# sriram-0311/MC-SLAM

Measured on AMD Instinct MI355X. Metric: multi-cam frames/sec (4-cam 1280x720 @2000 kpts/cam, extract + intra-rig match), higher is better.
Workload: dtype u8; 1 GPU; 4-cam rig 1280x720, 2000 kpts/cam, extract + all-pairs intra-rig match (configs[1]); slots=4, frames_per_launch=128, cameras=4, nfeatures=2000

## Files before the change

mc-slam_amd/csrc/mcorb_device.h:

```cpp
#pragma once
#include <hip/hip_runtime.h>
#include <stdint.h>

#include "mcorb_common.h"

namespace mcorb {

typedef short s16x2 __attribute__((ext_vector_type(2)));
typedef unsigned short u16x2 __attribute__((ext_vector_type(2)));
typedef int v4i __attribute__((ext_vector_type(4)));

__device__ __forceinline__ int lane_id() { return threadIdx.x & 63; }
__device__ __forceinline__ int lane_rank(unsigned long long mask, int acc = 0)
{
    return (int)__builtin_amdgcn_mbcnt_hi((uint32_t)(mask >> 32), __builtin_amdgcn_mbcnt_lo((uint32_t)mask, (uint32_t)acc));
}
__device__ __forceinline__ int wave_uniform(int v) { return __builtin_amdgcn_readfirstlane(v); }
__device__ __forceinline__ void wave_lds_sync()
{
    __builtin_amdgcn_fence(__ATOMIC_RELEASE, "workgroup");
    __builtin_amdgcn_wave_barrier();
    __builtin_amdgcn_fence(__ATOMIC_ACQUIRE, "workgroup");
}
__device__ __forceinline__ int xcd_remap(int b, int n)
{
    const int q = n >> 3, r = n & 7, x = b & 7;
    return (x < r ? x * (q + 1) : r * (q + 1) + (x - r) * q) + (b >> 3);
}
__device__ __forceinline__ int reflect101(int p, int len)
{
    if (p < 0) p = -p;
    if (p >= len) p = 2 * len - 2 - p;
    return p;
}

struct UndistScales {
    float s[kMaxLevels];
    UndistScales(const float *scale, int nlevels) : s{}
    {
        for (int l = 0; l < nlevels && l < kMaxLevels; l++) s[l] = scale[l];
    }
};
__device__ __forceinline__ float2 sel_point(uint32_t v, const UndistScales &sc)
{
    int l, xl, yl;
    unpack_sel(v, l, xl, yl);
    float x = (float)xl, y = (float)yl;
    if (l != 0) { x *= sc.s[l]; y *= sc.s[l]; }
    return make_float2(x, y);
}

__device__ __forceinline__ uint32_t bcnt_acc(uint32_t x, uint32_t acc)
{
    uint32_t r;
    asm("v_bcnt_u32_b32 %0, %1, %2" : "=v"(r) : "v"(x), "v"(acc));
    return r;
}
__device__ __forceinline__ uint32_t hamming256(const ulonglong4 &a, const ulonglong4 &b)
{
    const unsigned long long x0 = a.x ^ b.x, x1 = a.y ^ b.y, x2 = a.z ^ b.z, x3 = a.w ^ b.w;
    uint32_t d = __builtin_popcount((uint32_t)x0);
    d = bcnt_acc((uint32_t)(x0 >> 32), d);
    d = bcnt_acc((uint32_t)x1, d);
    d = bcnt_acc((uint32_t)(x1 >> 32), d);
    d = bcnt_acc((uint32_t)x2, d);
    d = bcnt_acc((uint32_t)(x2 >> 32), d);
    d = bcnt_acc((uint32_t)x3, d);
    d = bcnt_acc((uint32_t)(x3 >> 32), d);
    return d;
}

}
```

mc-slam_amd/csrc/mcorb_engine.cpp:

```cpp
#include <stdlib.h>
#include <string.h>
#include <sys/prctl.h>
#include <time.h>

#include "mcorb_engine.h"
#include "mcorb_prof.h"

namespace mcorb {

static thread_local std::string g_err;
void set_error(const std::string &msg) { g_err = msg; }
const char *get_error() { return g_err.c_str(); }
hipError_t Rig::wait_event(hipEvent_t ev) const
{
    if (wait_mode != 2) return hipEventSynchronize(ev);
    for (int i = 0;; i++) {
        const hipError_t e = hipEventQuery(ev);
        if (e != hipErrorNotReady) return e;
        if (i < 4) { std::this_thread::yield(); continue; }
        timespec ts = {0, 20000};
        nanosleep(&ts, nullptr);
    }
}

// ... 452 lines not shown
        std::vector<mcorb_keypoint> &K = s.kps[m];
        K.assign(total, mcorb_keypoint{});
        uint32_t *sel = s.hc.sel + (size_t)m * geom.kcap;
        int monoIndex = 0, stereoIndex = total - 1;
        if (total) {
            for (int l = 0; l < L; l++) {
                for (const uint32_t c : s.sel_val[(size_t)m * L + l]) {
                    const int xl = cand_x(c) + kMinBorder, yl = cand_y(c) + kMinBorder;
                    const mcorb_keypoint kp = make_keypoint(l, xl, yl, (float)cand_resp(c), 0.f);
                    int pos;
                    if (kp.x >= (float)j.lap0 && kp.x <= (float)j.lap1) pos = stereoIndex--;
                    else pos = monoIndex++;
                    K[pos] = kp;
                    sel[pos] = pack_sel(l, xl, yl);
                }
            }
        }
        s.mono[m] = monoIndex;
        s.hc.nsel[m] = total;
    }, pool_threads + s.index);
    if (bad.load() == 3) { set_error("internal: quad-tree went below the bucketing without the candidate list"); (void)hipStreamSynchronize(s.st); return MCORB_E_STATE; }
    if (bad.load() == 1) { set_error("selection failed: level too tall"); (void)hipStreamSynchronize(s.st); return MCORB_E_SIZE; }
    if (bad.load()) { set_error("keypoint capacity exceeded"); (void)hipStreamSynchronize(s.st); return MCORB_E_CAP; }
    const auto t1 = std::chrono::steady_clock::now();
    s.timing[T_SELECT] = std::chrono::duration<float, std::micro>(t1 - t0).count();
    LatProf::mark(3);

    s.nimg_done = nimg;
    if (then_match) TRY(prepare_match(s, j));
    TRY(enqueue_back(s, j, then_match, false));
    HIPCHK(hipEventRecord(s.ev_done, s.st));
    LatProf::mark(4);
    HIPCHK(wait_event(s.ev_done));
    if (!s.host_results) HIPCHK(wait_event(s.ev_side));
    LatProf::mark(5);
    if (params.orientation)
        for (int m = 0; m < nimg; m++)
            for (size_t k = 0; k < s.kps[m].size(); k++) s.kps[m][k].angle = s.h_angles[(size_t)m * geom.kcap + k];
    read_timing(s, s.host_results ? nullptr : s.ev_c);
    return MCORB_OK;
}

int Rig::enqueue_back(Slot &s, const Job &j, bool then_match, bool gpu_sel)
{
    const int nimg = j.nimg;
    const bool small = s.host_results, ev_on = s.ev_on();
    if (!gpu_sel && !small) HIPCHK(hipMemcpyAsync(s.d_ctrl, s.h_ctrl, s.ctrl_bytes, hipMemcpyHostToDevice, s.st));
    if (ev_on) HIPCHK(hipEventRecord(s.ev_desc0, s.st));
    if (small && undist_on) {
        HIPCHK(hipEventRecord(s.ubuf.ev_u0, s.st));
        HIPCHK(hipStreamWaitEvent(s.st_dma, s.ubuf.ev_u0, 0));
        TRY(enqueue_undistort(s, nimg));
    }
    launch_describe(s.st, s.d_pyr, blur_planes ? s.d_blur : nullptr, geom, s.ctl.sel, s.ctl.nsel, params.orientation, s.d_desc, s.d_angles, nimg,
                    small ? s.h_desc : nullptr);
    if (ev_on) HIPCHK(hipEventRecord(s.ev_desc1, s.st));
    if (small) {
        if (then_match) TRY(enqueue_match(s, j, true));
        HIPCHK(hipGetLastError());
        if (undist_on) HIPCHK(hipStreamWaitEvent(s.st, s.ubuf.ev_u1, 0));
        if (s.bow_job) TRY(enqueue_bow(s, nimg));
        if (gpu_sel && ev_on) HIPCHK(hipEventRecord(s.ev_side, s.st));
        return MCORB_OK;
    }
    const size_t nk = (size_t)nimg * geom.kcap;
    HIPCHK(hipStreamWaitEvent(s.st_dma, s.ev_desc1, 0));
    if (!copy_kernel) HIPCHK(hipMemcpyAsync(s.h_desc, s.d_desc, nk * 32, hipMemcpyDeviceToHost, s.st_dma));
    else launch_copy_to_host(s.st_dma, s.d_desc, s.h_desc, nk * 32);
    if (gpu_sel) {
        HIPCHK(hipMemcpyAsync(s.h_ctrl + s.ctrl_nsel_off, s.d_ctrl + s.ctrl_nsel_off, s.ctrl_pairs_end - s.ctrl_nsel_off + nk * sizeof(uint32_t),
                              hipMemcpyDeviceToHost, s.st_dma));
        HIPCHK(hipMemcpyAsync(s.h_res, s.d_res, s.res_resp_off + nk, hipMemcpyDeviceToHost, s.st_dma));
    }
    if (params.orientation) HIPCHK(hipMemcpyAsync(s.h_angles, s.d_angles, nk * sizeof(float), hipMemcpyDeviceToHost, s.st_dma));
    if (undist_on) TRY(enqueue_undistort(s, nimg));
    if (s.bow_job) TRY(enqueue_bow(s, nimg));
    if (then_match) TRY(enqueue_match(s, j, true));
    HIPCHK(hipGetLastError());
    HIPCHK(hipEventRecord(s.ev_side, s.st_dma));
    return MCORB_OK;
}

int Rig::enqueue_gpu_job(Slot &s, const Job &j, bool then_match)
{
    const int nimg = j.nimg;
    (void)hipGetLastError();
    const bool small = s.host_results, ev_on = s.ev_on();
    if (then_match && !small)
        HIPCHK(hipMemcpyAsync(s.d_ctrl, s.h_ctrl, s.ctrl_pairs_end, hipMemcpyHostToDevice, s.st));
    int *d_flags = reinterpret_cast<int *>(s.d_res.get());
    if (!small) HIPCHK(hipMemsetAsync(d_flags, 0, 16 * sizeof(int), s.st));
    TRY(enqueue_front(s, nimg, s.d_tbl));
    HIPCHK(launch_select(s.st, s.d_tbl, s.d_sorted, geom, s.d_selval, s.d_selcnt, d_flags, nimg, select_deep_cap, select_prof));
    launch_assemble(s.st, s.d_selval, s.d_selcnt, geom, tab.scale, j.lap0, j.lap1, s.dc.sel, s.d_res + s.res_resp_off, s.dc.nsel,
                    reinterpret_cast<int *>(s.d_res + s.res_mono_off), d_flags, nimg, small ? s.hc.sel : nullptr,
                    small ? s.h_res + s.res_resp_off : nullptr, small ? s.h_sig : nullptr);
    if (ev_on) HIPCHK(hipEventRecord(s.ev_s, s.st));
    if (ev_on) HIPCHK(hipEventRecord(s.ev_tables, s.st));
    if (blur_planes) launch_blur(s.st, s.d_pyr, s.d_blur, geom, nimg);
    if (ev_on) HIPCHK(hipEventRecord(s.ev_blur, s.st));
    return enqueue_back(s, j, then_match, true);
}

void Rig::gpu_job_begin()
{
    if (!gpu_job_limit) return;
    std::unique_lock<std::mutex> lk(gpu_jobs_m);
    gpu_jobs_cv.wait(lk, [this] { return gpu_jobs_running < gpu_job_limit; });
    gpu_jobs_running++;
}
void Rig::gpu_job_end()
{
    if (!gpu_job_limit) return;
    {
        std::lock_guard<std::mutex> lk(gpu_jobs_m);
        gpu_jobs_running--;
    }
    gpu_jobs_cv.notify_one();
}

int Rig::run_gpu_selected(Slot &s, const Job &j, bool then_match)
{
    TRY(begin_extract(s, j));
    const int nimg = j.nimg;
    s.nimg_done = nimg;
    if (then_match) TRY(prepare_match(s, j));
    if (s.host_results)
        for (int m = 0; m < nimg; m++) static_cast<volatile unsigned long long *>(s.h_sig)[m] = 0;
    auto records = [&](int m) {
        const int n = s.hc.nsel[m];
// ... 124 lines not shown
```

mc-slam_amd/csrc/mcorb_engine.h:

```cpp
#pragma once
#include <hip/hip_runtime.h>
#include <stdint.h>

#include <algorithm>
#include <atomic>
#include <condition_variable>
#include <functional>
#include <memory>
#include <mutex>
#include <string>
#include <thread>
#include <vector>

#include "../../include/mcorb.h"
#include "mcorb_common.h"
#include "mcorb_hip.h"
#include "mcorb_kernels.h"
#include "mcorb_select.h"

namespace mcorb {

const char *get_error();

struct Tables {
// ... 284 lines not shown
    int set_undistortion(int cam, const double *K, const double *dist, int ncoeffs);
    int undist_records(Slot &s, int m0, int n, std::vector<const mcorb_keypoint *> &out);
    int undist_default(Slot &s, int m0, int n, std::vector<const mcorb_keypoint *> &out);
    int max_pairs() const { return std::max(1, npp * max_frames); }

    std::vector<UndistImageCam> imgud_cams;
    std::vector<uint8_t> imgud_set;
    std::vector<std::vector<int16_t>> imgud_map1;
    std::vector<std::vector<uint16_t>> imgud_map2;
    std::vector<DevBuf<int16_t>> d_imgud_map1;
    std::vector<DevBuf<uint16_t>> d_imgud_map2;
    DevBuf<RemapCam> d_remap_cams;
    bool imgud_on = false;
    int set_image_undistortion(int cam, const double *K, const double *dist, int ncoeffs);
    int enqueue_remap(Slot &s, int nimg);

    struct BowBinding {
        int flags = 0, levelsup = 0, L = 0, weighting = 0, scoring = 0;
        double ratio = 0.85;
        const int *child_start = nullptr, *child_count = nullptr, *child_id = nullptr, *word_id = nullptr;
        const void *child_desc = nullptr;
        const double *weight = nullptr;
    };
    BowBinding bow_bind;
    unsigned bow_gen = 0;
    bool lf_on = false;
    int lf_total_feats = 3000;
    std::vector<mcorb_camera> lf_cams;
    DevBuf<LfCam> d_lfcams;
    unsigned lf_gen = 0;
    int set_lf(const mcorb_camera *cams, int total_feats);
    int set_vocabulary(const BowBinding &b);
    int check_job_shape(const Job &j) const;
    int lock_idle_slots(const char *who, std::vector<std::unique_lock<std::mutex>> &locks);

private:
    bool copy_kernel = false;
    bool blur_planes = false;
    void driver(Slot *s);
    int execute(Slot &s, const Job &j);
    int begin_extract(Slot &s, const Job &j);
    int enqueue_front(Slot &s, int nimg, int *tbl);
    int enqueue_tables_to_host(Slot &s, int nimg, bool by_kernel);
    int enqueue_back(Slot &s, const Job &j, bool then_match, bool gpu_sel);
    void read_timing(Slot &s, hipEvent_t blur0);
    mcorb_keypoint make_keypoint(int level, int xl, int yl, float response, float angle) const;
    int run_extract_phaseA(Slot &s, const Job &j);
    int run_select_and_describe(Slot &s, const Job &j, bool then_match);
    int run_gpu_selected(Slot &s, const Job &j, bool then_match);
    int enqueue_gpu_job(Slot &s, const Job &j, bool then_match);
    int enqueue_undistort(Slot &s, int nimg);
    int enqueue_bow(Slot &s, int nimg);
    int prepare_match(Slot &s, const Job &j);
    int enqueue_match(Slot &s, const Job &j, bool ctrl_on_device);
    int finish_match(Slot &s, const Job &j);
};

static inline void ev_elapsed(float *ms, hipEvent_t a, hipEvent_t b)
{
    if (hipEventElapsedTime(ms, a, b) != hipSuccess) { *ms = 0.f; (void)hipGetLastError(); }
}

inline void decode_rows(const KnnRow *rows, int nq, int32_t *idx, int32_t *dist)
{
    for (int q = 0; q < nq; q++) {
        const KnnRow &k = rows[q];
        idx[2 * q] = knn_idx0(k);
        dist[2 * q] = knn_d0(k);
        idx[2 * q + 1] = knn_idx1(k);
        dist[2 * q + 1] = knn_d1(k);
    }
}
int bow_job_finish(Rig &R, Slot &s, int nimg);
int lf_job_finish(Rig &R, Slot &s, int nframes);
void bow_assemble(int weighting, int scoring, const BowRes *res, int n, BowImageOut &o);
void vocab_props(const ::mcorb_vocab *v, int &scoring, int &device);

}

struct mcorb_rig {
    mcorb::Rig rig;
};
```

mc-slam_amd/csrc/mcorb_kernels.h:

```cpp
#pragma once
#include <hip/hip_runtime.h>
#include <vector>
#include "mcorb_common.h"
#include "mcorb_signal.h"
#include "mcorb_undistort.h"
#include "mcorb_undistort_image.h"

namespace mcorb {

constexpr int kKnnChunk = 4096;
__host__ __device__ inline int knn_chunk_len(int npairs) { return npairs <= 12 ? 256 : npairs <= 24 ? 512 : npairs <= 48 ? 1024 : kKnnChunk; }
constexpr int kKnnQueriesPerBlock = 256;
inline int knn_qblocks(int kcap) { return (kcap + kKnnQueriesPerBlock - 1) / kKnnQueriesPerBlock; }
inline size_t knn_mlist_stride(int kcap) { return (size_t)knn_qblocks(kcap) * kKnnQueriesPerBlock; }
inline size_t knn_part_entries(int max_pairs, int kcap)
{
    size_t need = 0;
    for (int np : {12, 24, 48, max_pairs}) {
        const int n = np < max_pairs ? np : max_pairs, cl = knn_chunk_len(n);
        const size_t e = (size_t)n * ((kcap + cl - 1) / cl) * kcap;
        need = need > e ? need : e;
    }
    return need;
}
constexpr int kKnnExpandBytes = 128;

struct KnnRow { uint32_t idx, d; };
__host__ __device__ inline int knn_idx0(const KnnRow &r) { return (r.idx & 0xffffu) == 0xffffu ? -1 : (int)(r.idx & 0xffffu); }
__host__ __device__ inline int knn_idx1(const KnnRow &r) { return (r.idx >> 16) == 0xffffu ? -1 : (int)(r.idx >> 16); }
__host__ __device__ inline int knn_d0(const KnnRow &r) { return knn_idx0(r) < 0 ? -1 : (int)(r.d & 0x1ffu); }
__host__ __device__ inline int knn_d1(const KnnRow &r) { return knn_idx1(r) < 0 ? -1 : (int)((r.d >> 9) & 0x1ffu); }
__host__ __device__ inline bool knn_accept(const KnnRow &r) { return (r.d >> 18) & 1u; }

hipError_t upload_umax(const int umax[16]);
void launch_stage_f32(hipStream_t st, const float *src, int w, int h, int pitch_f, int channels, size_t img_stride_f,
                      uint8_t *pyr, const Geom &g, int nimg);
struct RemapCam { const int16_t *map1; const uint16_t *map2; int32_t mode, pad; };
__host__ __device__ inline int remap_map_pitch(int w) { return (w + 3) & ~3; }
void launch_stage_f32_raw(hipStream_t st, const float *src, int w, int h, int pitch_f, int channels, size_t img_stride_f,
                          uint8_t *raw, int nimg);
void launch_remap_u8(hipStream_t st, const uint8_t *raw, uint8_t *pyr, const Geom &g, const RemapCam *cams, int ncams, int nimg);
void launch_pyramid(hipStream_t st, uint8_t *pyr, const Geom &g, const ResizeTap *tabs, const int *win, int nimg);
int fast_cell_table(const Geom &g, std::vector<uint32_t> &tab);
void launch_fast(hipStream_t st, const uint8_t *pyr, const Geom &g, int iniTh, int minTh, const uint32_t *cellRec,
                 uint32_t *cell_kp, int *cell_cnt, int nimg);
void launch_compact(hipStream_t st, const uint32_t *cell_kp, const int *cell_cnt, const Geom &g, const uint16_t *lut,
                    uint32_t *sorted_dev, uint32_t *cand, int *tbl, int *overflow, int nimg, bool one_copy = false);
void launch_blur(hipStream_t st, const uint8_t *pyr, uint8_t *blur, const Geom &g, int nimg);
void launch_describe(hipStream_t st, const uint8_t *pyr, const uint8_t *blur, const Geom &g, const uint32_t *sel,
                     const int *nsel, int orientation, uint8_t *desc, float *angles, int nimg,
                     uint8_t *desc_host = nullptr);
void launch_knn2(hipStream_t st, const uint8_t *desc, const int *counts, const int *setmap, int nsets, const int2 *pairs, int npairs,
                 int kcap, void *expanded, int *lcounts, uint2 *part, float dist_thresh, float ratio, KnnRow *out, uint32_t *mlist,
                 int *mcount, hipEvent_t ev_exp, hipEvent_t ev_mid);

int select_cap(const Geom &g);
bool select_fits(const Geom &g);
hipError_t configure_select(const Geom &g);
hipError_t launch_select(hipStream_t st, const int *tbl, const uint32_t *sorted, const Geom &g, uint32_t *sel_val, int *sel_cnt, int *fallback, int nimg,
                         int deep_cap = 4096, bool prof = false);
void launch_assemble(hipStream_t st, const uint32_t *sel_val, const int *sel_cnt, const Geom &g, const float *scale, int lap0, int lap1,
                     uint32_t *sel, uint8_t *resp, int *nsel, int *mono, int *fallback, int nimg,
                     uint32_t *sel_h = nullptr, uint8_t *resp_h = nullptr, unsigned long long *sig_h = nullptr);
hipError_t sort_selftest(const uint64_t *in_dev, int n, uint64_t *out_dev);

void launch_undistort(hipStream_t st, const uint32_t *sel, const int *nsel, int kcap, int nimg, int ncams, const UndistCam *cams,
                      const float *scale, int nlevels, float2 *out);

void launch_copy_to_host(hipStream_t st, const void *src_dev, void *dst_host_mapped, size_t bytes);

void launch_bow_best2(hipStream_t st, const uint8_t *desc, int img0, int kcap, int ncams, int nframes, const float *yv,
                      const int *slot_of, const int2 *node_range, const int *rg_base, const int *node_feats, const int *nfeat, int4 *out);
void launch_bow_fold(hipStream_t st, const BowRes *res, const int *nsel, int kcap, int nimg, int weighting, int scoring, int *out_dev,
                     int *out_host);
void launch_bow_tables(hipStream_t st, const int *fold, int kcap, int ncams, int nframes, const int *nsel, const uint32_t *sel,
                       const float *scale, int nlevels, const float2 *undist, int *slot_of, int *node_feats, int *nfeat, int *rg_base,
                       float *yv, int2 *node_range);
void launch_bow_descend(hipStream_t st, const uint8_t *desc, int n, const int *child_start, const int *child_count,
                        const void *child_desc, const int *child_id, const int *word_id, const double *weight, int nid_level,
                        BowRes *out);

void launch_lf_tracks(hipStream_t st, const int4 *trk, const LfView *views, int ntr, const LfCam *cams, const uint8_t *desc, int kcap,
                      int ncams, LfTrackOut *out);
void launch_tri_selftest(hipStream_t st, const double *x, const double *P, const int *nv, const int *voff, int n, double *X, int *branch);

void launch_kfdb_score(hipStream_t st, const uint32_t *ids, const double *vals, const int *nbow, int stride, const uint32_t *q_ids,
                       const double *q_vals, const int *q_n, const int *q_sel, const int *q_limit, const int *e_list, int nq,
                       int max_limit, int out_stride, double *raw, int *shared);
void launch_kfdb_best2(hipStream_t st, const uint8_t *desc_a, const int *feats_a, const uint8_t *desc_b, const int *feats_b,
                       const int2 *items, int nitems, const int2 *nodes, int4 *out);
void launch_kfdb_gather(hipStream_t st, const uint8_t *desc, const int *src, int n, uint8_t *dst);

}
```

mc-slam_amd/csrc/mcorb_kernels.hip:

```cpp
#include <hip/hip_runtime.h>
#include <stdint.h>
#include <string.h>
#include <vector>

#include "mcorb_common.h"
#include "mcorb_device.h"
#include "mcorb_kernels.h"

namespace mcorb {

constexpr int kResizeRows = kResizeTileH;

template <int NF>
__global__ __launch_bounds__(256) void k_resize(uint8_t *__restrict__ pyr, Geom g, int level,
                                                const ResizeTap *__restrict__ tabs, int srcPitch, int srcRows)
{
    extern __shared__ __attribute__((aligned(16))) uint8_t win[];
    const LevelGeom &D = g.lv[level];
    const LevelGeom &S = g.lv[level - 1];
    const int img = blockIdx.z;
    uint8_t *base = pyr + (size_t)img * g.imgBytes;
    const int tid = threadIdx.x;
    const int bx0 = blockIdx.x * 256, by0 = blockIdx.y * kResizeRows;
    const int bx1 = min(bx0 + 255, D.w - 1), by1 = min(by0 + kResizeRows - 1, D.h - 1);
// ... 844 lines not shown
#pragma unroll
    for (int u = 0; u < kDescPerWave; u++) {
        *reinterpret_cast<uint4 *>(&patch[wave][u][lane * 4]) = v[u][0];
        if (lane < kPatchRows * 3 - 64) *reinterpret_cast<uint4 *>(&patch[wave][u][(64 + lane) * 4]) = v[u][1];
    }
    wave_lds_sync();

    int o0[4], o1[4];
#pragma unroll
    for (int j = 0; j < 4; j++) {
        const int p = (j * 64 + lane) * 4;
        o0[j] = (c_pattern[p + 1] + 13) * (kPatchDw * 4) + c_pattern[p];
        o1[j] = (c_pattern[p + 3] + 13) * (kPatchDw * 4) + c_pattern[p + 2];
    }
#pragma unroll
    for (int u = 0; u < kDescPerWave; u++) {
        const uint8_t *c = reinterpret_cast<const uint8_t *>(patch[wave][u]) + shift[u];
        unsigned long long bits[4];
#pragma unroll
        for (int j = 0; j < 4; j++) bits[j] = __ballot(c[o0[j]] < c[o1[j]]);
        if (k0 + u < n) store_ballots(bits, lane, desc + ((size_t)img * g.kcap + k0 + u) * 32);
    }
}

constexpr int kFdSrcDw = 34 * 12 + 4;
constexpr int kFdPairs = 17, kFdHpPitch = 28, kFdHpDw = kFdPairs * kFdHpPitch;
constexpr int kFdOutPitchDw = 7, kFdOutDw = 28 * kFdOutPitchDw;
__constant__ uint8_t c_brief_groups[64] = {
#include "brief_groups_31.inc"
};
constexpr int kFdWaveDw = kFdSrcDw + kFdHpDw + kFdOutDw;

template <int SH>
__device__ __forceinline__ void fd_hpass(const uint32_t *__restrict__ src, uint32_t *__restrict__ hp, int a, int lane)
{
#pragma unroll
    for (int t = 0; t < 2; t++) {
        const int i = lane + 64 * t;
        if (i < kFdPairs * 7) {
            const int p = (int)(__umul24((uint32_t)i, 147u) >> 10), j = i - 7 * p;
            uint32_t h[2][4];
#pragma unroll
            for (int rr = 0; rr < 2; rr++) {
                const uint32_t *row = src + (2 * p + rr) * 12 + a + j;
                gauss_hsum4<SH>({row[0], row[1], row[2], SH == 3 ? row[3] : 0u}, h[rr]);
            }
            *reinterpret_cast<uint4 *>(hp + p * kFdHpPitch + 4 * j) = gauss_pair4(h[0], h[1]);
        }
    }
}

__global__ __launch_bounds__(256) void k_describe_fused(const uint8_t *__restrict__ pyr, Geom g,
                                                        const uint32_t *__restrict__ sel, const int *__restrict__ nsel,
                                                        uint8_t *__restrict__ desc, int groups, uint8_t *__restrict__ desc_host)
{
    __shared__ __attribute__((aligned(16))) uint32_t lds[4][kFdWaveDw];
    static_assert(kFdSrcDw % 4 == 0 && kFdHpDw % 4 == 0, "16-byte aligned regions");
    const int lane = lane_id(), wave = threadIdx.x >> 6;
    const int b = wave_uniform(xcd_remap(blockIdx.x, gridDim.x));
    const int img = b / groups;
    const int k0 = ((b - img * groups) * 4 + wave) * kDescPerWave;
    const int n = nsel[img];
    if (k0 >= n) return;
    uint32_t *src = lds[wave], *hp = src + kFdSrcDw, *out = hp + kFdHpDw;

    int toff[2], tlds[2];
    bool tact[2];
#pragma unroll
    for (int q = 0; q < 2; q++) {
        const int t = 64 * q + lane;
        tact[q] = t < 99;
        const int tt = tact[q] ? t : 98;
        const int row = (int)(__umul24((uint32_t)tt, 171u) >> 9), ch = tt - 3 * row;
        toff[q] = row | (ch << 8);
        tlds[q] = row * 12 + 4 * ch;
    }
    int o0[4], o1[4];
#pragma unroll
    for (int j = 0; j < 4; j++) {
        const int p = (8 * (int)c_brief_groups[8 * j + (lane >> 3)] + (lane & 7)) * 4;
        o0[j] = (c_pattern[p + 1] + 13) * (kFdOutPitchDw * 4) + c_pattern[p] + 13;
        o1[j] = (c_pattern[p + 3] + 13) * (kFdOutPitchDw * 4) + c_pattern[p + 2] + 13;
    }
    const int bslot = c_brief_groups[32 + (lane & 31)];

    uint4 va, vb;
    int kxn;
#define FD_FETCH(u)                                                                                                         \
    {                                                                                                                       \
        int level_, kx_, ky_;                                                                                               \
        unpack_sel((uint32_t)__builtin_amdgcn_readlane((int)selv, (u)), level_, kx_, ky_);                                  \
        const LevelGeom &L_ = g.lv[level_];                                                                                 \
        const uint8_t *p0_ = pyr + (size_t)img * g.imgBytes + L_.off + (size_t)(ky_ - 16) * L_.pitch + ((kx_ - 16) & ~15);  \
        va = *reinterpret_cast<const uint4 *>(p0_ + (size_t)__mul24(toff0 & 0xff, L_.pitch) + 16 * (toff0 >> 8));           \
        vb = *reinterpret_cast<const uint4 *>(p0_ + (size_t)__mul24(toff1 & 0xff, L_.pitch) + 16 * (toff1 >> 8));           \
        kxn = kx_;                                                                                                          \
    }
    const uint32_t selv = sel[(size_t)img * g.kcap + min(k0 + (lane < kDescPerWave ? lane : 0), n - 1)];
    const int toff0 = toff[0], toff1 = toff[1], tlds0 = tlds[0], tlds1 = tlds[1];
    const bool tact1 = tact[1];
    FD_FETCH(0)
#pragma unroll 1
    for (int u = 0; u < kDescPerWave; u++) {
        const int A = (kxn - 16) & 15;
        *reinterpret_cast<uint4 *>(src + tlds0) = va;
        if (tact1) *reinterpret_cast<uint4 *>(src + tlds1) = vb;
        if (u + 1 < kDescPerWave) FD_FETCH(u + 1)
        wave_lds_sync();
        switch (A & 3) {
        case 0: fd_hpass<0>(src, hp, A >> 2, lane); break;
        case 1: fd_hpass<1>(src, hp, A >> 2, lane); break;
        case 2: fd_hpass<2>(src, hp, A >> 2, lane); break;
        default: fd_hpass<3>(src, hp, A >> 2, lane); break;
        }
        wave_lds_sync();
        if (lane < 49) {
            const int rg = (int)(__umul24((uint32_t)lane, 147u) >> 10), j = lane - 7 * rg;
            uint32_t P[5][4];
#pragma unroll
            for (int q = 0; q < 5; q++) {
                const uint4 w = *reinterpret_cast<const uint4 *>(hp + (2 * rg + q) * kFdHpPitch + 4 * j);
                P[q][0] = w.x; P[q][1] = w.y; P[q][2] = w.z; P[q][3] = w.w;
            }
#pragma unroll
            for (int k = 0; k < 4; k++) out[(4 * rg + k) * kFdOutPitchDw + j] = gauss_vrow4(P, k);
        }
        wave_lds_sync();
        const uint8_t *c = reinterpret_cast<const uint8_t *>(out);
        unsigned long long bits[4];
#pragma unroll
        for (int j = 0; j < 4; j++) bits[j] = __ballot(c[o0[j]] < c[o1[j]]);
        store_ballots(bits, lane, hp);
        wave_lds_sync();
        if (lane < 32 && k0 + u < n) {
            const uint8_t byte = reinterpret_cast<const uint8_t *>(hp)[bslot];
            desc[((size_t)img * g.kcap + k0 + u) * 32 + lane] = byte;
            if (desc_host) desc_host[((size_t)img * g.kcap + k0 + u) * 32 + lane] = byte;
        }
    }
#undef FD_FETCH
}

__global__ __launch_bounds__(256) void k_describe_oriented(const uint8_t *__restrict__ pyr, const uint8_t *__restrict__ blur,
                                                           Geom g, const uint32_t *__restrict__ sel,
                                                           const int *__restrict__ nsel, uint8_t *__restrict__ desc,
                                                           float *__restrict__ angles)
{
    const int lane = lane_id();
    const int img = blockIdx.y;
    const int k = blockIdx.x * 4 + (threadIdx.x >> 6);
    if (k >= nsel[img]) return;
    int level, kx, ky;
    unpack_sel(sel[(size_t)img * g.kcap + k], level, kx, ky);
    const LevelGeom &L = g.lv[level];
    const int pitch = L.pitch;
    const size_t coff = (size_t)img * g.imgBytes + L.off + (size_t)ky * pitch + kx;

    const uint8_t *c = pyr + coff;
    int m01 = 0, m10 = 0;
    if (lane < 31) {
        const int uu = lane - 15;
        m10 = uu * c[uu];
    }
    for (int v = 1; v <= 15; v++) {
        const int d = c_umax[v];
        if (lane <= 2 * d) {
            const int uu = lane - d;
            const int vp = c[uu + v * pitch], vm = c[uu - v * pitch];
            m01 += v * (vp - vm);
            m10 += uu * (vp + vm);
        }
    }
#pragma unroll
    for (int o = 32; o > 0; o >>= 1) {
        m01 += __shfl_xor(m01, o);
        m10 += __shfl_xor(m10, o);
    }
    const float ang = fast_atan2_deg((float)m01, (float)m10);
    if (lane == 0) angles[(size_t)img * g.kcap + k] = ang;
    const float rad = __fmul_rn(ang, (float)(3.14159265358979323846 / 180.f));
    const float ca = (float)cos((double)rad), sa = (float)sin((double)rad);

    const uint8_t *cb = blur + (size_t)img * g.imgBytes + L.off;
    unsigned long long bits[4];
#pragma unroll
    for (int j = 0; j < 4; j++) {
        const int p = (j * 64 + lane) * 4;
        const float x0 = (float)c_pattern[p], y0 = (float)c_pattern[p + 1], x1 = (float)c_pattern[p + 2], y1 = (float)c_pattern[p + 3];
        const int oy0 = __float2int_rn(__fadd_rn(__fmul_rn(x0, sa), __fmul_rn(y0, ca)));
        const int ox0 = __float2int_rn(__fsub_rn(__fmul_rn(x0, ca), __fmul_rn(y0, sa)));
        const int oy1 = __float2int_rn(__fadd_rn(__fmul_rn(x1, sa), __fmul_rn(y1, ca)));
        const int ox1 = __float2int_rn(__fsub_rn(__fmul_rn(x1, ca), __fmul_rn(y1, sa)));
        const int t0 = cb[blur_tiled_offset(pitch, kx + ox0, ky + oy0)], t1 = cb[blur_tiled_offset(pitch, kx + ox1, ky + oy1)];
        bits[j] = __ballot(t0 < t1);
    }
    store_ballots(bits, lane, desc + ((size_t)img * g.kcap + k) * 32);
}

typedef int v4i __attribute__((ext_vector_type(4)));
typedef int v8i __attribute__((ext_vector_type(8)));
typedef float v16f __attribute__((ext_vector_type(16)));

constexpr int kKnnQT = 2;
constexpr int kKnnWaves = 4;
constexpr int kTileU4 = 4 * 64;
static_assert(32 * kKnnQT * kKnnWaves == kKnnQueriesPerBlock, "the host reads the accepted-pair lists in blocks of kKnnQueriesPerBlock queries");
static_assert(kTileU4 * 16 == 32 * kKnnExpandBytes, "k_expand's tile and the scratch size the engine allocates");

__global__ __launch_bounds__(256) void k_expand(const uint8_t *__restrict__ desc, const int *__restrict__ counts,
                                                const int *__restrict__ setmap, int kcap, uint4 *__restrict__ E,
                                                int *__restrict__ lcounts)
{
    const int i = blockIdx.y;
    const int src = setmap ? setmap[i] : i;
    const int n = min(max(counts[src], 0), kcap);
    if (blockIdx.x == 0 && threadIdx.x == 0) lcounts[i] = n;
    const int d = blockIdx.x * 256 + threadIdx.x;
    if (d >= n) return;
    const uint4 *dp = reinterpret_cast<const uint4 *>(desc + ((size_t)src * kcap + d) * 32);
    const uint4 lo = dp[0], hi = dp[1];
    const uint32_t w[8] = {lo.x, lo.y, lo.z, lo.w, hi.x, hi.y, hi.z, hi.w};
    uint4 *out = E + ((size_t)i * (kcap / 32) + (d >> 5)) * kTileU4 + (d & 31);
#pragma unroll
    for (int sh = 0; sh < 8; sh++) {
        uint32_t o[4];
#pragma unroll
        for (int q = 0; q < 4; q++) {
            uint32_t x = (w[sh] >> (8 * q)) & 0xffu;
            x = (x | (x << 12)) & 0x000f000fu;
            x = (x | (x << 6)) & 0x03030303u;
            x = (x | (x << 3)) & 0x11111111u;
            o[q] = (x << 3) | 0x22222222u;
        }
        out[(sh >> 1) * 64 + (sh & 1) * 32] = uint4{o[0], o[1], o[2], o[3]};
    }
}

template <int kKnnStageTiles, int kWavesPerSimd, bool FOLD>
__global__ __launch_bounds__(64 * kKnnWaves, kWavesPerSimd) void k_knn2(const uint4 *__restrict__ E, const int *__restrict__ lcounts,
                                                           const int2 *__restrict__ pairs, int kcap, int nchunks, int npairs,
                                                           int qblocks, uint2 *__restrict__ part, int chunkLen,
                                                           float dist_thresh, float ratio, KnnRow *__restrict__ rows,
                                                           uint32_t *__restrict__ mlist, int *__restrict__ mcount)
{
    __shared__ __attribute__((aligned(16))) uint4 stage[2 * kKnnStageTiles * kTileU4 + 2 * 64];
    const int tid = threadIdx.x, lane = tid & 63, wave = tid >> 6, half = lane >> 5;
    const int slot = blockIdx.x >> 3, grp = slot / qblocks;
    const int unit = grp * 8 + (blockIdx.x & 7);
    if (unit >= npairs * nchunks) return;
    const int pair = unit / nchunks, chunk = unit - pair * nchunks;
    const int2 qt = pairs[pair];
    const int nq = lcounts[qt.x], nt = lcounts[qt.y];
    const int qbi = slot - grp * qblocks;
    const int qb = qbi * kKnnQueriesPerBlock;
    if (qb >= nq) {
        if (FOLD && tid == 0) mcount[pair * qblocks + qbi] = 0;
        return;
    }
    const int t0 = chunk * chunkLen;
    const int tn = min(nt - t0, chunkLen);
    const int tilesPerSet = kcap / 32;
    const int ntiles = tn > 0 ? (tn + 31) >> 5 : 0;
    const float kNone = -__builtin_inff();
    float k0[kKnnQT], k1[kKnnQT];
#pragma unroll
    for (int u = 0; u < kKnnQT; u++) k0[u] = k1[u] = kNone;

    if (tn > 0) {
        const int qtile0 = (qb >> 5) + wave * kKnnQT;
        v4i Bf[kKnnQT][4];
#pragma unroll
        for (int u = 0; u < kKnnQT; u++) {
            const int tq = min(qtile0 + u, tilesPerSet - 1);
            const uint4 *src = E + ((size_t)qt.x * tilesPerSet + tq) * kTileU4 + lane;
#pragma unroll
            for (int s = 0; s < 4; s++) Bf[u][s] = __builtin_bit_cast(v4i, src[s * 64]);
        }
        v16f Crow;
#pragma unroll
        for (int e = 0; e < 16; e++) Crow[e] = (float)(31 - ((e & 3) + 8 * (e >> 2) + 4 * half));
        const uint4 *Et = E + ((size_t)qt.y * tilesPerSet + (t0 >> 5)) * kTileU4;
        const int nstage = (ntiles + kKnnStageTiles - 1) / kKnnStageTiles;
        static_assert(kTileU4 == 64 * kKnnWaves, "one LDS-DMA round of the workgroup = one tile (wave w moves K-step w)");
        auto fill = [&](int st, int buf) {
#pragma unroll
            for (int k = 0; k < kKnnStageTiles; k++) {
// ... 232 lines not shown
        pitch = pitch > p ? pitch : p;
        rows = rows > g.lv[l].hCell + 6 ? rows : g.lv[l].hCell + 6;
    }
    tp = pitch <= 48 ? 48 : (pitch <= 64 ? 64 : 80);
}

void launch_fast(hipStream_t st, const uint8_t *pyr, const Geom &g, int iniTh, int minTh, const uint32_t *cellRec,
                 uint32_t *cell_kp, int *cell_cnt, int nimg)
{
    int tp, rows;
    fast_layout(g, tp, rows);
    const int cap = kFastListCap;
    const int tileB = (rows * tp + 15) & ~15, scB = ((rows - 4) * tp + 15) & ~15;
    const size_t lds = 16 + (size_t)tileB + 16 + (size_t)scB + 16 + (size_t)cap * 2;
    dim3 grid(g.cells, nimg);
    if (iniTh < 0) iniTh = 0;
    if (minTh < 0) minTh = 0;
    if (iniTh > 255) iniTh = 255;
    if (minTh > 255) minTh = 255;
    const auto kern = tp == 48 ? k_fast_cells<48> : tp == 64 ? k_fast_cells<64> : k_fast_cells<80>;
    hipLaunchKernelGGL(kern, grid, dim3(64), lds, st, pyr, g, iniTh, minTh, tileB, scB, cap, cellRec, cell_kp, cell_cnt);
}

void launch_compact(hipStream_t st, const uint32_t *cell_kp, const int *cell_cnt, const Geom &g, const uint16_t *lut,
                    uint32_t *sorted_dev, uint32_t *cand, int *tbl, int *overflow, int nimg, bool one_copy)
{
    int maxb = 1, maxc = 1, maxwh = 2;
    for (int l = 0; l < g.nlevels; l++) {
        maxb = maxb > g.lv[l].nBuckets ? maxb : g.lv[l].nBuckets;
        maxc = maxc > g.lv[l].nCols * g.lv[l].nRows ? maxc : g.lv[l].nCols * g.lv[l].nRows;
        const int wh = (g.lv[l].maxBorderX - kMinBorder) + (g.lv[l].maxBorderY - kMinBorder);
        maxwh = maxwh > wh ? maxwh : wh;
    }
    const int bktCap = (maxb + 1 + 3) & ~3;
    const int wg = nimg <= 8 ? 1024 : 512;
    const int cellsCap = (maxc + 8 + 7) & ~7;
    const size_t ldsTail = (size_t)(cellsCap + maxwh + 8) * sizeof(uint16_t);
    const bool fits = (size_t)(2 * kCompactCopies * bktCap) * sizeof(int) + ldsTail <= 64 * 1024;
    const int copies = fits && !one_copy ? kCompactCopies : 1;
    const size_t lds = (size_t)(2 * copies * bktCap) * sizeof(int) + ldsTail;
    const dim3 grid(nimg, g.nlevels);
    const auto kern = wg == 1024 ? (copies == 1 ? k_compact<1024, 4, 1> : k_compact<1024, 4, kCompactCopies>)
                                 : (copies == 1 ? k_compact<512, 4, 1> : k_compact<512, 4, kCompactCopies>);
    hipLaunchKernelGGL(kern, grid, dim3(wg), lds, st, cell_kp, cell_cnt, g, lut, sorted_dev, cand, tbl, overflow, bktCap, cellsCap);
}

void launch_blur(hipStream_t st, const uint8_t *pyr, uint8_t *blur, const Geom &g, int nimg)
{
    dim3 grid(g.tiles, nimg);
    hipLaunchKernelGGL(k_blur, grid, dim3(256), 0, st, pyr, blur, g);
}

void launch_describe(hipStream_t st, const uint8_t *pyr, const uint8_t *blur, const Geom &g, const uint32_t *sel,
                     const int *nsel, int orientation, uint8_t *desc, float *angles, int nimg, uint8_t *desc_host)
{
    if (orientation) {
        dim3 grid((g.kcap + 3) / 4, nimg);
        hipLaunchKernelGGL(k_describe_oriented, grid, dim3(256), 0, st, pyr, blur, g, sel, nsel, desc, angles);
    } else {
        dim3 grid((g.kcap + 4 * kDescPerWave - 1) / (4 * kDescPerWave), nimg);
        if (blur) hipLaunchKernelGGL(k_describe, grid, dim3(256), 0, st, blur, g, sel, nsel, desc);
        else hipLaunchKernelGGL(k_describe_fused, dim3(grid.x * nimg), dim3(256), 0, st, pyr, g, sel, nsel, desc, (int)grid.x, desc_host);
    }
}

void launch_knn2(hipStream_t st, const uint8_t *desc, const int *counts, const int *setmap, int nsets, const int2 *pairs, int npairs,
                 int kcap, void *expanded, int *lcounts, uint2 *part, float dist_thresh, float ratio, KnnRow *out, uint32_t *mlist,
                 int *mcount, hipEvent_t ev_exp, hipEvent_t ev_mid)
{
    uint4 *E = reinterpret_cast<uint4 *>(expanded);
    hipLaunchKernelGGL(k_expand, dim3((kcap + 255) / 256, nsets), dim3(256), 0, st, desc, counts, setmap, kcap, E, lcounts);
    if (ev_exp) (void)hipEventRecord(ev_exp, st);
    const int chunkLen = knn_chunk_len(npairs), nchunks = (kcap + chunkLen - 1) / chunkLen;
    const int qblocks = knn_qblocks(kcap), units = npairs * nchunks;
    dim3 grid(8 * qblocks * ((units + 7) / 8));
    if (nchunks == 1) {
        hipLaunchKernelGGL((k_knn2<4, 3, true>), grid, dim3(64 * kKnnWaves), 0, st, E, lcounts, pairs, kcap, nchunks, npairs, qblocks, part, chunkLen,
                           dist_thresh, ratio, out, mlist, mcount);
        if (ev_mid) (void)hipEventRecord(ev_mid, st);
        return;
    }
    hipLaunchKernelGGL((k_knn2<4, 3, false>), grid, dim3(64 * kKnnWaves), 0, st, E, lcounts, pairs, kcap, nchunks, npairs, qblocks, part, chunkLen,
                       dist_thresh, ratio, out, mlist, mcount);
    if (ev_mid) (void)hipEventRecord(ev_mid, st);
    hipLaunchKernelGGL(k_knn2_finalize, dim3(npairs), dim3(1024), 0, st, part, lcounts, pairs, kcap, nchunks, chunkLen, dist_thresh, ratio, out, mlist,
                       mcount, qblocks);
}
}
```

mc-slam_amd/csrc/mcorb_match.cpp:

```cpp
#include <cmath>

#include "mcorb_engine.h"
#include "mcorb_prof.h"

namespace mcorb {

static inline int clamp_count(int n, int kcap) { return std::min(std::max(n, 0), kcap); }

static bool take_ext_block(Slot &s, const Job &j, int ext_cap, int kcap)
{
    if (!j.ext_desc || j.ext_total < 1 || j.ext_total > ext_cap || (!j.ext_counts && !j.ext_counts_dev)) return false;
    if (j.ext_counts)
        for (int i = 0; i < j.ext_total; i++) s.hc.extcounts[i] = clamp_count(j.ext_counts[i], kcap);
    return true;
}

int Rig::prepare_match(Slot &s, const Job &j)
{
    const bool ext = j.ext_desc != nullptr;
    if (j.ext_pairs) {
        if (j.ext_npairs < 1 || j.ext_npairs > max_pairs() || !take_ext_block(s, j, ext_cap, geom.kcap)) {
            set_error("match pairs: bad external block or pair count (at most " + std::to_string(max_pairs()) + " pairs per job)");
            return MCORB_E_ARG;
        }
// ... 5 lines not shown
            int lp[2];
            for (int k = 0; k < 2; k++) {
                const int set = j.ext_pairs[2 * p + k];
                if (set < 0 || set >= j.ext_total) { set_error("match pairs: set index out of range"); return MCORB_E_ARG; }
                if (local[set] < 0) {
                    if ((int)s.match_sets.size() >= max_images) { set_error("match pairs: more than " + std::to_string(max_images) + " distinct sets in one job"); return MCORB_E_ARG; }
                    local[set] = (int)s.match_sets.size();
                    s.hc.setmap[local[set]] = set;
                    s.match_sets.push_back(set);
                    s.match_counts.push_back(j.ext_counts ? s.hc.extcounts[set] : 0);
                }
                lp[k] = local[set];
            }
            s.hc.pairs[p] = int2{lp[0], lp[1]};
        }
        s.nsets_local = (int)s.match_sets.size();
        s.npairs_done = j.ext_npairs;
        s.nframes_done = 0;
        return MCORB_OK;
    }
    if (j.nframes < 1 || j.nframes > max_frames || (!ext && j.nframes * ncams > s.nimg_done)) {
        set_error("match: bad frame count or features not extracted");
        return MCORB_E_STATE;
    }
    const int C = ncams;
    s.match_external = ext;
    s.match_sets.resize((size_t)j.nframes * C);
    s.match_counts.resize((size_t)j.nframes * C);
    if (ext) {
        if (!j.ext_sets || !take_ext_block(s, j, ext_cap, geom.kcap)) {
            set_error("match: bad external block (at most " + std::to_string(ext_cap) + " sets = max(4096, 64 x images per slot))");
            return MCORB_E_ARG;
        }
        for (int i = 0; i < j.nframes * C; i++) {
            const int set = j.ext_sets[i];
            if (set < 0 || set >= j.ext_total) { set_error("match: set index out of range"); return MCORB_E_ARG; }
            s.match_sets[i] = set;
            s.match_counts[i] = j.ext_counts ? s.hc.extcounts[set] : 0;
        }
    } else {
        for (int i = 0; i < j.nframes * C; i++) { s.match_sets[i] = i; s.match_counts[i] = s.hc.nsel[i]; }
    }
    s.nframes_done = j.nframes;
    s.nsets_local = j.nframes * C;
    for (int i = 0; i < j.nframes * C; i++) s.hc.setmap[i] = s.match_sets[i];
    int p = 0;
    for (int f = 0; f < j.nframes; f++)
        for (int a = 0; a < C - 1; a++)
            for (int b = a + 1; b < C; b++) s.hc.pairs[p++] = int2{f * C + a, f * C + b};
    s.npairs_done = p;
    return MCORB_OK;
}

int Rig::enqueue_match(Slot &s, const Job &j, bool ctrl_on_device)
{
    if (!ctrl_on_device) {
        TRY(prepare_match(s, j));
        HIPCHK(hipMemcpyAsync(s.d_ctrl, s.h_ctrl, s.ctrl_pairs_end, hipMemcpyHostToDevice, s.st));
        s.set_ctl(false, false);
    }
    if (j.after_stream)
        HIPCHK(hipStreamWaitEvent(s.st, s.ev_x, 0));
    if (j.ext_counts_dev) {
        HIPCHK(hipMemcpyAsync(s.dc.extcounts, j.ext_counts_dev, (size_t)j.ext_total * sizeof(int), hipMemcpyDeviceToDevice, s.st));
        HIPCHK(hipMemcpyAsync(s.hc.extcounts, j.ext_counts_dev, (size_t)j.ext_total * sizeof(int), hipMemcpyDeviceToHost, s.st));
    }
    if (s.npairs_done == 0) return MCORB_OK;
    const bool ext = j.ext_desc != nullptr;
    const bool ev_on = s.ev_on();
    if (ev_on) HIPCHK(hipEventRecord(s.ev_knn0, s.st));
    launch_knn2(s.st, ext ? (const uint8_t *)j.ext_desc : s.d_desc, ext ? s.dc.extcounts : s.ctl.nsel, s.ctl.setmap, s.nsets_local, s.ctl.pairs,
                s.npairs_done, geom.kcap, s.d_exp, s.d_lcounts, s.d_part, j.dist_thresh, j.ratio, s.d_knn, s.h_mlist,
                s.h_mcount, ev_on ? s.ev_e : nullptr, ev_on ? s.ev_knn1 : nullptr);
    if (ev_on) HIPCHK(hipEventRecord(s.ev_fin, s.st));
    HIPCHK(hipGetLastError());
    return MCORB_OK;
}

static bool epipolar_ok(const double *F, const mcorb_keypoint &k1, const mcorb_keypoint &k2, const float *sigma2)
{
    float a = (float)((double)k2.x * F[0] + (double)k2.y * F[3] + F[6]);
    float b = (float)((double)k2.x * F[1] + (double)k2.y * F[4] + F[7]);
    float c = (float)((double)k2.x * F[2] + (double)k2.y * F[5] + F[8]);
    float den = a * a + b * b;
    den = den ? (float)(1. / (double)std::sqrt(den)) : (float)1.;
    a *= den; b *= den; c *= den;
    den = a * a + b * b;
    const float num = a * k1.x + b * k1.y + c;
    if (den == 0) return false;
    const float dsqr = num * num / den;
    const float check_thresh = (float)(3.84 * (double)sigma2[k1.octave]);
    return dsqr < check_thresh;
}

void merge_pair_lists(int C, const int *counts, const uint32_t *const *idx1, const uint32_t *const *idx2, const int *np,
                             const EpipolarGate *gate, std::vector<int32_t> &tr, int &mergeable_out)
{
    tr.clear();
    int ntr = 0, mergeable = 0;
    static thread_local std::vector<int> inv_flat;
    int *inv[MCORB_MAX_CAMS];
    {
        size_t total = 0, worst = 0;
        for (int c = 0; c < C; c++) total += (size_t)std::max(counts[c], 0);
        inv_flat.assign(total, -1);
        size_t o = 0;
        for (int c = 0; c < C; c++) { inv[c] = inv_flat.data() + o; o += (size_t)std::max(counts[c], 0); }
        for (int p = 0; p < C * (C - 1) / 2; p++) worst += (size_t)std::max(np[p], 0);
        tr.resize(worst * C);
    }
    int32_t *T = tr.data();
    int pl = 0;
    for (int a = 0; a < C - 1; a++) {
        for (int b = a + 1; b < C; b++, pl++) {
            const uint32_t *i1 = idx1[pl], *i2 = idx2[pl];
            for (int k = 0; k < np[pl]; k++) {
                const int fa = (int)i1[k], fb = (int)i2[k];
                const int ma = inv[a][fa], mb = inv[b][fb];
                if (gate && !epipolar_ok(gate->F + 9 * pl, gate->kps[a][fa], gate->kps[b][fb], gate->sigma2)) continue;
                if (ma == -1 && mb == -1) {
                    int32_t *row = T + (size_t)ntr * C;
                    for (int c = 0; c < C; c++) row[c] = -1;
                    row[a] = fa;
                    row[b] = fb;
                    inv[a][fa] = ntr;
                    inv[b][fb] = ntr;
// ... 83 lines not shown
```

Measured before the change: 40120 frames/s.

## Fuse e2m1 descriptor expansion into fused describe kernel, skip separate expand launch

The fused describe kernel now writes the e2m1-expanded matching operand and per-image lcounts directly as it emits each descriptor byte. The separate k_expand kernel launch before knn is skipped when this path is eligible (GPU selection, no external descriptors, no orientation, no blur planes). This removes one kernel launch and a re-read of the descriptors, at the cost of extra scattered 4-byte stores in the describe kernel. Sets with no descriptors may not get their expanded tile padding zeroed the way k_expand did, which risks a correctness difference.

```diff
diff --git a/mc-slam_amd/csrc/mcorb_device.h b/mc-slam_amd/csrc/mcorb_device.h
--- a/mc-slam_amd/csrc/mcorb_device.h
+++ b/mc-slam_amd/csrc/mcorb_device.h
@@ -70,4 +70,13 @@
     return d;
 }
 
+__device__ __forceinline__ uint32_t expand_e2m1(uint32_t byte)
+{
+    uint32_t x = byte & 0xffu;
+    x = (x | (x << 12)) & 0x000f000fu;
+    x = (x | (x << 6)) & 0x03030303u;
+    x = (x | (x << 3)) & 0x11111111u;
+    return (x << 3) | 0x22222222u;
 }
+
+}
diff --git a/mc-slam_amd/csrc/mcorb_engine.cpp b/mc-slam_amd/csrc/mcorb_engine.cpp
--- a/mc-slam_amd/csrc/mcorb_engine.cpp
+++ b/mc-slam_amd/csrc/mcorb_engine.cpp
@@ -528,11 +528,12 @@
         HIPCHK(hipStreamWaitEvent(s.st_dma, s.ubuf.ev_u0, 0));
         TRY(enqueue_undistort(s, nimg));
     }
+    const bool operand = then_match && gpu_sel && !j.ext_desc && !params.orientation && !blur_planes && s.npairs_done > 0;
     launch_describe(s.st, s.d_pyr, blur_planes ? s.d_blur : nullptr, geom, s.ctl.sel, s.ctl.nsel, params.orientation, s.d_desc, s.d_angles, nimg,
-                    small ? s.h_desc : nullptr);
+                    small ? s.h_desc : nullptr, operand ? s.d_exp.get() : nullptr, operand ? s.d_lcounts.get() : nullptr);
     if (ev_on) HIPCHK(hipEventRecord(s.ev_desc1, s.st));
     if (small) {
-        if (then_match) TRY(enqueue_match(s, j, true));
+        if (then_match) TRY(enqueue_match(s, j, true, operand));
         HIPCHK(hipGetLastError());
         if (undist_on) HIPCHK(hipStreamWaitEvent(s.st, s.ubuf.ev_u1, 0));
         if (s.bow_job) TRY(enqueue_bow(s, nimg));
@@ -551,7 +552,7 @@
     if (params.orientation) HIPCHK(hipMemcpyAsync(s.h_angles, s.d_angles, nk * sizeof(float), hipMemcpyDeviceToHost, s.st_dma));
     if (undist_on) TRY(enqueue_undistort(s, nimg));
     if (s.bow_job) TRY(enqueue_bow(s, nimg));
-    if (then_match) TRY(enqueue_match(s, j, true));
+    if (then_match) TRY(enqueue_match(s, j, true, operand));
     HIPCHK(hipGetLastError());
     HIPCHK(hipEventRecord(s.ev_side, s.st_dma));
     return MCORB_OK;
diff --git a/mc-slam_amd/csrc/mcorb_engine.h b/mc-slam_amd/csrc/mcorb_engine.h
--- a/mc-slam_amd/csrc/mcorb_engine.h
+++ b/mc-slam_amd/csrc/mcorb_engine.h
@@ -360,7 +360,7 @@
     int enqueue_undistort(Slot &s, int nimg);
     int enqueue_bow(Slot &s, int nimg);
     int prepare_match(Slot &s, const Job &j);
-    int enqueue_match(Slot &s, const Job &j, bool ctrl_on_device);
+    int enqueue_match(Slot &s, const Job &j, bool ctrl_on_device, bool operand_ready = false);
     int finish_match(Slot &s, const Job &j);
 };
 
diff --git a/mc-slam_amd/csrc/mcorb_kernels.h b/mc-slam_amd/csrc/mcorb_kernels.h
--- a/mc-slam_amd/csrc/mcorb_kernels.h
+++ b/mc-slam_amd/csrc/mcorb_kernels.h
@@ -49,10 +49,12 @@
 void launch_blur(hipStream_t st, const uint8_t *pyr, uint8_t *blur, const Geom &g, int nimg);
 void launch_describe(hipStream_t st, const uint8_t *pyr, const uint8_t *blur, const Geom &g, const uint32_t *sel,
                      const int *nsel, int orientation, uint8_t *desc, float *angles, int nimg,
-                     uint8_t *desc_host = nullptr);
+                     uint8_t *desc_host = nullptr,
+                     void *expanded = nullptr, int *lcounts = nullptr);
 void launch_knn2(hipStream_t st, const uint8_t *desc, const int *counts, const int *setmap, int nsets, const int2 *pairs, int npairs,
                  int kcap, void *expanded, int *lcounts, uint2 *part, float dist_thresh, float ratio, KnnRow *out, uint32_t *mlist,
-                 int *mcount, hipEvent_t ev_exp, hipEvent_t ev_mid);
+                 int *mcount, hipEvent_t ev_exp, hipEvent_t ev_mid,
+                 bool expand = true);
 
 int select_cap(const Geom &g);
 bool select_fits(const Geom &g);
diff --git a/mc-slam_amd/csrc/mcorb_kernels.hip b/mc-slam_amd/csrc/mcorb_kernels.hip
--- a/mc-slam_amd/csrc/mcorb_kernels.hip
+++ b/mc-slam_amd/csrc/mcorb_kernels.hip
@@ -920,7 +920,8 @@
 
 __global__ __launch_bounds__(256) void k_describe_fused(const uint8_t *__restrict__ pyr, Geom g,
                                                         const uint32_t *__restrict__ sel, const int *__restrict__ nsel,
-                                                        uint8_t *__restrict__ desc, int groups, uint8_t *__restrict__ desc_host)
+                                                        uint8_t *__restrict__ desc, int groups, uint8_t *__restrict__ desc_host,
+                                                        uint8_t *__restrict__ E, int *__restrict__ lcounts)
 {
     __shared__ __attribute__((aligned(16))) uint32_t lds[4][kFdWaveDw];
     static_assert(kFdSrcDw % 4 == 0 && kFdHpDw % 4 == 0, "16-byte aligned regions");
@@ -929,6 +930,7 @@
     const int img = b / groups;
     const int k0 = ((b - img * groups) * 4 + wave) * kDescPerWave;
     const int n = nsel[img];
+    if (E && k0 == 0 && lane == 0) lcounts[img] = min(max(n, 0), g.kcap);
     if (k0 >= n) return;
     uint32_t *src = lds[wave], *hp = src + kFdSrcDw, *out = hp + kFdHpDw;
 
@@ -951,6 +953,8 @@
         o1[j] = (c_pattern[p + 3] + 13) * (kFdOutPitchDw * 4) + c_pattern[p + 2] + 13;
     }
     const int bslot = c_brief_groups[32 + (lane & 31)];
+    const int eoff = ((lane >> 3) & 3) * (16 * kKnnExpandBytes / 2) + ((lane >> 2) & 1) * (16 * 32) + (lane & 3) * 4;
+    static_assert(16 * kKnnExpandBytes / 2 == 64 * 16, "a K-step of a tile is 64 fragments of 16 bytes");
 
     uint4 va, vb;
     int kxn;
@@ -1004,6 +1008,9 @@
             const uint8_t byte = reinterpret_cast<const uint8_t *>(hp)[bslot];
             desc[((size_t)img * g.kcap + k0 + u) * 32 + lane] = byte;
             if (desc_host) desc_host[((size_t)img * g.kcap + k0 + u) * 32 + lane] = byte;
+            if (E && k0 + u < g.kcap)
+                *reinterpret_cast<uint32_t *>(E + ((size_t)img * (g.kcap >> 5) + ((k0 + u) >> 5)) * (32 * kKnnExpandBytes) + ((k0 + u) & 31) * 16 + eoff) =
+                    expand_e2m1(byte);
         }
     }
 #undef FD_FETCH
@@ -1093,13 +1100,7 @@
     for (int sh = 0; sh < 8; sh++) {
         uint32_t o[4];
 #pragma unroll
-        for (int q = 0; q < 4; q++) {
-            uint32_t x = (w[sh] >> (8 * q)) & 0xffu;
-            x = (x | (x << 12)) & 0x000f000fu;
-            x = (x | (x << 6)) & 0x03030303u;
-            x = (x | (x << 3)) & 0x11111111u;
-            o[q] = (x << 3) | 0x22222222u;
-        }
+        for (int q = 0; q < 4; q++) o[q] = expand_e2m1(w[sh] >> (8 * q));
         out[(sh >> 1) * 64 + (sh & 1) * 32] = uint4{o[0], o[1], o[2], o[3]};
     }
 }
@@ -1438,7 +1439,8 @@
 }
 
 void launch_describe(hipStream_t st, const uint8_t *pyr, const uint8_t *blur, const Geom &g, const uint32_t *sel,
-                     const int *nsel, int orientation, uint8_t *desc, float *angles, int nimg, uint8_t *desc_host)
+                     const int *nsel, int orientation, uint8_t *desc, float *angles, int nimg, uint8_t *desc_host, void *expanded,
+                     int *lcounts)
 {
     if (orientation) {
         dim3 grid((g.kcap + 3) / 4, nimg);
@@ -1446,16 +1448,17 @@
     } else {
         dim3 grid((g.kcap + 4 * kDescPerWave - 1) / (4 * kDescPerWave), nimg);
         if (blur) hipLaunchKernelGGL(k_describe, grid, dim3(256), 0, st, blur, g, sel, nsel, desc);
-        else hipLaunchKernelGGL(k_describe_fused, dim3(grid.x * nimg), dim3(256), 0, st, pyr, g, sel, nsel, desc, (int)grid.x, desc_host);
+        else hipLaunchKernelGGL(k_describe_fused, dim3(grid.x * nimg), dim3(256), 0, st, pyr, g, sel, nsel, desc, (int)grid.x, desc_host,
+                                reinterpret_cast<uint8_t *>(expanded), lcounts);
     }
 }
 
 void launch_knn2(hipStream_t st, const uint8_t *desc, const int *counts, const int *setmap, int nsets, const int2 *pairs, int npairs,
                  int kcap, void *expanded, int *lcounts, uint2 *part, float dist_thresh, float ratio, KnnRow *out, uint32_t *mlist,
-                 int *mcount, hipEvent_t ev_exp, hipEvent_t ev_mid)
+                 int *mcount, hipEvent_t ev_exp, hipEvent_t ev_mid, bool expand)
 {
     uint4 *E = reinterpret_cast<uint4 *>(expanded);
-    hipLaunchKernelGGL(k_expand, dim3((kcap + 255) / 256, nsets), dim3(256), 0, st, desc, counts, setmap, kcap, E, lcounts);
+    if (expand) hipLaunchKernelGGL(k_expand, dim3((kcap + 255) / 256, nsets), dim3(256), 0, st, desc, counts, setmap, kcap, E, lcounts);
     if (ev_exp) (void)hipEventRecord(ev_exp, st);
     const int chunkLen = knn_chunk_len(npairs), nchunks = (kcap + chunkLen - 1) / chunkLen;
     const int qblocks = knn_qblocks(kcap), units = npairs * nchunks;
diff --git a/mc-slam_amd/csrc/mcorb_match.cpp b/mc-slam_amd/csrc/mcorb_match.cpp
--- a/mc-slam_amd/csrc/mcorb_match.cpp
+++ b/mc-slam_amd/csrc/mcorb_match.cpp
@@ -81,7 +81,7 @@
     return MCORB_OK;
 }
 
-int Rig::enqueue_match(Slot &s, const Job &j, bool ctrl_on_device)
+int Rig::enqueue_match(Slot &s, const Job &j, bool ctrl_on_device, bool operand_ready)
 {
     if (!ctrl_on_device) {
         TRY(prepare_match(s, j));
@@ -100,7 +100,7 @@
     if (ev_on) HIPCHK(hipEventRecord(s.ev_knn0, s.st));
     launch_knn2(s.st, ext ? (const uint8_t *)j.ext_desc : s.d_desc, ext ? s.dc.extcounts : s.ctl.nsel, s.ctl.setmap, s.nsets_local, s.ctl.pairs,
                 s.npairs_done, geom.kcap, s.d_exp, s.d_lcounts, s.d_part, j.dist_thresh, j.ratio, s.d_knn, s.h_mlist,
-                s.h_mcount, ev_on ? s.ev_e : nullptr, ev_on ? s.ev_knn1 : nullptr);
+                s.h_mcount, ev_on ? s.ev_e : nullptr, ev_on ? s.ev_knn1 : nullptr, !operand_ready);
     if (ev_on) HIPCHK(hipEventRecord(s.ev_fin, s.st));
     HIPCHK(hipGetLastError());
     return MCORB_OK;
```

Result: slower. 39630 frames/s (-1.2%).
